# kkromberg/SpeechRecognition

Measured on AMD Instinct MI355X. Metric: frames/sec scored+decoded, higher is better.
Workload: dtype f64

## Files before the change

include/srgpu.h:

```cpp
#ifndef SRGPU_H
#define SRGPU_H

#include <stddef.h>
#include <stdint.h>

#ifdef __cplusplus
extern "C" {
#endif

#if defined(__GNUC__)
#define SR_API __attribute__((visibility("default")))
#else
#define SR_API
#endif

#define SR_ABI_VERSION 4
SR_API int sr_abi_version(void);

#define SR_OK 0
#define SR_EINVAL (-1)
#define SR_EHIP (-2)
#define SR_ENODEV (-3)
#define SR_ELIMIT (-4)
#define SR_ENOMEM (-5)
// ... 192 lines not shown
                                        double posterior_floor, uint32_t max_items, const uint32_t* trans,
                                        const uint64_t* trans_off, double* out_cost, uint16_t* out_count,
                                        uint16_t* out_state, double* out_weight);
SR_API int sr_bigram_mmi_statistics_corpus(sr_model* m, sr_corpus* c, sr_bigram* b, int gmm_kernel, double scale,
                                           double posterior_floor, int max_approx, const uint32_t* trans,
                                           const uint64_t* trans_off, double* out_num_cost, double* out_den_cost,
                                           double* num_mean_acc, double* num_mean_w, double* num_var_acc, double* num_var_w,
                                           double* den_mean_acc, double* den_mean_w, double* den_var_acc, double* den_var_w);


SR_API int sr_bigram_word_lattice_corpus(sr_model* m, sr_corpus* c, sr_bigram* b, int gmm_kernel, double lattice_beam, uint64_t cap,
                                         uint64_t* out_arc_off, double* out_best, uint32_t* out_word, uint32_t* out_hist,
                                         uint32_t* out_pred, uint32_t* out_first, uint32_t* out_last, double* out_fwd, double* out_bwd,
                                         double* out_am);
SR_API int sr_bigram_lattice_nbest(uint32_t n_frames, uint64_t n_arcs, const uint32_t* word, const uint32_t* hist,
                                   const uint32_t* first, const uint32_t* last, const double* am, uint32_t n_words,
                                   uint32_t silence_word, const float* lm, double lm_scale, uint32_t n_best, uint32_t* out_words,
                                   uint64_t words_cap, uint64_t* out_off, double* out_cost, uint32_t* out_count);

typedef struct sr_bigram_stream sr_bigram_stream;
SR_API int sr_bigram_stream_open(sr_model* m, sr_bigram* b, const sr_bigram_params* p, uint32_t max_streams, uint64_t max_frames,
                                 sr_bigram_stream** out);
SR_API int sr_bigram_stream_begin(sr_bigram_stream* s, uint32_t* id);
SR_API int sr_bigram_stream_push(sr_bigram_stream* s, uint32_t n, const uint32_t* ids, const float* feats, const uint64_t* frame_off);
SR_API int sr_bigram_stream_partial(sr_bigram_stream* s, uint32_t id, uint32_t* out_word, float* out_score, uint32_t* out_time,
                                    uint32_t cap, uint32_t* count, uint64_t* frames);
SR_API int sr_bigram_stream_end(sr_bigram_stream* s, uint32_t id, uint32_t* out_word, float* out_score, uint32_t* out_time,
                                uint32_t cap, uint32_t* count);
SR_API int sr_bigram_stream_destroy(sr_bigram_stream* s);

SR_API int sr_probe_fp16_denormals(int device, int* preserved);
SR_API int sr_probe_fp16_accumulation(int device, int* within_model, double* worst_ratio);

typedef struct {
  double gmm_ms;
  uint64_t gmm_launches;
  double gmm_flops;
  double search_ms;
  uint64_t search_launches;
  double search_bytes;
  uint64_t frames;
  uint64_t refined_pairs;
  uint64_t refined_densities;
  double prefilter_ms;
  double refine_ms;
} sr_profile;
SR_API int sr_profile_enable(sr_model* m, int on);
SR_API int sr_profile_reset(sr_model* m);
SR_API int sr_profile_read(sr_model* m, sr_profile* out);

#ifdef __cplusplus
}
#endif
#endif
```

speechrecognition_amd/capi.py:

```python
from __future__ import annotations

import ctypes as C
import os

import numpy as np

HERE = os.path.dirname(os.path.abspath(__file__))
LIB_PATH = os.environ.get("SRGPU_LIB") or os.path.join(HERE, "libsrgpu.so")

GMM_MFMA, GMM_EXACT, GMM_PREFILTER, GMM_DEFAULT = 0, 1, 2, 3
POOL_GLOBAL, POOL_MIXTURE, POOL_NONE = 0, 1, 2
SEARCH_GENERAL_KERNEL = 1
SEARCH_SLOT_KERNEL = 2
BIGRAM_DENSE_STATES = 1
BIGRAM_GLOBAL_STATES = 2
SR_ECORRUPT = -7
SR_ABI_VERSION = 4

SYMBOLS = [
    "sr_abi_version", "sr_model_trim",
    "sr_last_error", "sr_device_count", "sr_model_create", "sr_model_load_mixset", "sr_model_destroy", "sr_model_info",
    "sr_corpus_upload", "sr_corpus_upload_async", "sr_corpus_wait", "sr_corpus_destroy", "sr_shard_utterances", "sr_recognize_batch_multi", "sr_score_corpus", "sr_score_frames", "sr_lexicon_create",
    "sr_lexicon_destroy", "sr_lexicon_describe", "sr_recognize_corpus", "sr_traceback_corpus", "sr_traceback_words", "sr_recognize_batch", "sr_align_corpus", "sr_align_corpus_pruned", "sr_path_scores_corpus", "sr_model_create_from_statistics", "sr_model_create_from_accumulated", "sr_mixset_write", "sr_model_set_tying", "sr_model_tying_info", "sr_model_topology", "sr_accumulate_corpus",
    "sr_state_posteriors_corpus", "sr_baum_welch_corpus", "sr_word_posteriors_corpus", "sr_recognize_confidence_corpus",
    "sr_net_occupancies_corpus", "sr_mmi_statistics_corpus", "sr_model_create_from_mmi_statistics",
    "sr_smbr_max_positions", "sr_net_accuracies_corpus", "sr_smbr_statistics_corpus",
    "sr_word_lattice_corpus", "sr_lattice_nbest",
    "sr_fmllr_statistics_corpus", "sr_fmllr_statistics_bw_corpus", "sr_fmllr_estimate", "sr_corpus_transform",
    "sr_bigram_create", "sr_bigram_destroy", "sr_bigram_describe", "sr_recognize_bigram_corpus",
    "sr_bigram_word_posteriors_corpus", "sr_recognize_bigram_confidence_corpus",
    "sr_bigram_occupancies_corpus", "sr_bigram_mmi_statistics_corpus",
    "sr_bigram_word_lattice_corpus", "sr_bigram_lattice_nbest",
    "sr_stream_open", "sr_stream_begin", "sr_stream_push", "sr_stream_partial", "sr_stream_end", "sr_stream_destroy",
    "sr_bigram_stream_open", "sr_bigram_stream_begin", "sr_bigram_stream_push", "sr_bigram_stream_partial", "sr_bigram_stream_end",
    "sr_bigram_stream_destroy",
    "sr_probe_fp16_denormals", "sr_probe_fp16_accumulation",
    "sr_profile_enable", "sr_profile_reset", "sr_profile_read",
]


class SrError(RuntimeError):
    def __init__(self, code, msg):
        super().__init__(f"libsrgpu error {code}: {msg}")
        self.code = code


def smbr_max_positions():
    n = C.c_uint32()
    _check(lib().sr_smbr_max_positions(C.byref(n)))
    return n.value


class SearchParams(C.Structure):
    _fields_ = [("am_threshold", C.c_double), ("word_penalty", C.c_double), ("gmm_kernel", C.c_int), ("flags", C.c_int)]


class BigramParams(C.Structure):
    _fields_ = [("acoustic_pruning", C.c_float), ("lm_pruning", C.c_float), ("gmm_kernel", C.c_int), ("max_word_ends", C.c_uint32), ("flags", C.c_int)]


class Profile(C.Structure):
    _fields_ = [("gmm_ms", C.c_double), ("gmm_launches", C.c_uint64), ("gmm_flops", C.c_double),
                ("search_ms", C.c_double), ("search_launches", C.c_uint64), ("search_bytes", C.c_double),
                ("frames", C.c_uint64), ("refined_pairs", C.c_uint64), ("refined_densities", C.c_uint64),
                ("prefilter_ms", C.c_double), ("refine_ms", C.c_double)]


_lib = None

# ... 49 lines not shown
        L.sr_recognize_confidence_corpus.argtypes = [vp, vp, vp, C.POINTER(SearchParams), dbl, vp, vp, vp, vp, vp]
        L.sr_net_occupancies_corpus.argtypes = [vp, vp, vp, C.POINTER(SearchParams), dbl, dbl, u32, vp, vp, vp, vp, vp, vp]
        L.sr_mmi_statistics_corpus.argtypes = [vp, vp, vp, C.POINTER(SearchParams), dbl, dbl, i32, vp, vp] + [vp] * 10
        L.sr_smbr_max_positions.argtypes = [vp]
        L.sr_net_accuracies_corpus.argtypes = [vp, vp, vp, C.POINTER(SearchParams), dbl, dbl, u32, vp, vp, vp, vp, vp, vp]
        L.sr_smbr_statistics_corpus.argtypes = [vp, vp, vp, C.POINTER(SearchParams), dbl, dbl, i32, vp] + [vp] * 10
        L.sr_model_create_from_mmi_statistics.argtypes = [vp] + [vp] * 8 + [dbl, dbl, dbl, C.POINTER(vp)]
        L.sr_word_lattice_corpus.argtypes = [vp, vp, vp, C.POINTER(SearchParams), dbl, u64, vp, vp, vp, vp, vp, vp, vp, vp]
        L.sr_lattice_nbest.argtypes = [u32, u64, vp, vp, vp, vp, u32, u32, vp, u64, vp, vp, C.POINTER(u32)]
        L.sr_bigram_create.argtypes = [vp, u32, vp, vp, u32, vp, vp, C.POINTER(vp)]
        L.sr_bigram_destroy.argtypes = [vp]
        L.sr_bigram_describe.argtypes = [vp, C.c_char_p, C.c_size_t]
        L.sr_recognize_bigram_corpus.argtypes = [vp, vp, vp, C.POINTER(BigramParams), vp, vp, vp, vp]
        L.sr_bigram_word_posteriors_corpus.argtypes = [vp, vp, vp, i32, dbl, dbl, u32, vp, vp, vp, vp]
        L.sr_bigram_occupancies_corpus.argtypes = [vp, vp, vp, i32, dbl, dbl, u32, vp, vp, vp, vp, vp, vp]
        L.sr_bigram_mmi_statistics_corpus.argtypes = [vp, vp, vp, i32, dbl, dbl, i32, vp, vp] + [vp] * 10
        L.sr_recognize_bigram_confidence_corpus.argtypes = [vp, vp, vp, C.POINTER(BigramParams), dbl, vp, vp, vp, vp, vp]
        L.sr_bigram_word_lattice_corpus.argtypes = [vp, vp, vp, i32, dbl, u64] + [vp] * 10
        L.sr_bigram_lattice_nbest.argtypes = [u32, u64, vp, vp, vp, vp, vp, u32, u32, vp, dbl, u32, vp, u64, vp, vp, C.POINTER(u32)]
        L.sr_stream_open.argtypes = [vp, vp, C.POINTER(SearchParams), u32, u64, C.POINTER(vp)]
        L.sr_stream_begin.argtypes = [vp, C.POINTER(u32)]
        L.sr_stream_push.argtypes = [vp, u32, vp, vp, vp]
        L.sr_stream_partial.argtypes = [vp, u32, vp, u32, C.POINTER(u32), C.POINTER(u64)]
        L.sr_stream_end.argtypes = [vp, u32, vp, u32, C.POINTER(u32), vp, vp, vp]
        L.sr_stream_destroy.argtypes = [vp]
        L.sr_bigram_stream_open.argtypes = [vp, vp, C.POINTER(BigramParams), u32, u64, C.POINTER(vp)]
        L.sr_bigram_stream_begin.argtypes = [vp, C.POINTER(u32)]
        L.sr_bigram_stream_push.argtypes = [vp, u32, vp, vp, vp]
        L.sr_bigram_stream_partial.argtypes = [vp, u32, vp, vp, vp, u32, C.POINTER(u32), C.POINTER(u64)]
        L.sr_bigram_stream_end.argtypes = [vp, u32, vp, vp, vp, u32, C.POINTER(u32)]
        L.sr_bigram_stream_destroy.argtypes = [vp]
        L.sr_probe_fp16_denormals.argtypes = [i32, C.POINTER(i32)]
        L.sr_probe_fp16_accumulation.argtypes = [i32, C.POINTER(i32), C.POINTER(dbl)]
        L.sr_profile_enable.argtypes = [vp, i32]
        L.sr_profile_reset.argtypes = [vp]
        L.sr_profile_read.argtypes = [vp, C.POINTER(Profile)]
        _lib = L
    return _lib


def _check(rc):
    if rc != 0:
        raise SrError(rc, lib().sr_last_error().decode(errors="replace"))


def device_count():
    n = C.c_int(0)
    _check(lib().sr_device_count(C.byref(n)))
    return n.value


def _ptr(a):
    return a.ctypes.data if a is not None else None


class Model:

    def __init__(self, handle):
        self.h = handle
        d, s, c = C.c_uint32(), C.c_uint32(), C.c_uint64()
        _check(lib().sr_model_info(self.h, C.byref(d), C.byref(s), C.byref(c)))
        self.dim, self.n_states, self.n_densities = d.value, s.value, c.value

    @classmethod
    def from_mixset(cls, path, dim, pooling=POOL_NONE, max_approx=True, device=0):
        h = C.c_void_p()
# ... 50 lines not shown
        self.close()

    def score_frames(self, feats, kernel=GMM_PREFILTER):
        feats = np.ascontiguousarray(feats, dtype=np.float32)
        out = np.empty((feats.shape[0], self.n_states), dtype=np.float64)
        _check(lib().sr_score_frames(self.h, _ptr(feats), feats.shape[0], kernel, _ptr(out)))
        return out

    def upload(self, feats, frame_off, asynchronous=False):
        return Corpus(self, feats, frame_off, asynchronous)

    def recognize_batch(self, lexicon, feats, frame_off, am_threshold, word_penalty, kernel=GMM_PREFILTER):
        feats = np.ascontiguousarray(feats, dtype=np.float32)
        frame_off = np.ascontiguousarray(frame_off, dtype=np.uint64)
        n = len(frame_off) - 1
        words = np.zeros(max(int(frame_off[-1]), 1), dtype=np.uint32)
        woff = np.zeros(n + 1, dtype=np.uint64)
        sp = SearchParams(am_threshold, word_penalty, kernel, 0)
        _check(lib().sr_recognize_batch(self.h, lexicon.h, C.byref(sp), _ptr(feats), _ptr(frame_off), n, _ptr(words), _ptr(woff)))
        return words[: int(woff[-1])].copy(), woff

    def lexicon(self, word_off, automaton, silence_idx, tdp, silence_state):
        return Lexicon(self, word_off, automaton, silence_idx, tdp, silence_state)

    def bigram(self, word_off, mixtures, silence_word, lm, tdp):
        return Bigram(self, word_off, mixtures, silence_word, lm, tdp)

    def stream(self, lexicon, am_threshold, word_penalty, kernel=GMM_PREFILTER, max_streams=1, max_frames=65535):
        return Stream(self, lexicon, am_threshold, word_penalty, kernel, max_streams, max_frames)

    def bigram_stream(self, bigram, acoustic_pruning=None, lm_pruning=None, kernel=GMM_PREFILTER, max_streams=1, max_frames=65535):
        return BigramStream(self, bigram, FLT_MAX if acoustic_pruning is None else acoustic_pruning,
                            FLT_MAX if lm_pruning is None else lm_pruning, kernel, max_streams, max_frames)

    def profile(self, on=True):
        _check(lib().sr_profile_enable(self.h, int(on)))
        _check(lib().sr_profile_reset(self.h))

    def profile_read(self):
        p = Profile()
        _check(lib().sr_profile_read(self.h, C.byref(p)))
        return {k: getattr(p, k) for k, _ in Profile._fields_}


FLT_MAX = float(np.finfo(np.float32).max)


class Bigram:

    def __init__(self, model, word_off, mixtures, silence_word, lm, tdp):
        self.model = model
        word_off = np.ascontiguousarray(word_off, dtype=np.uint32)
        mixtures = np.ascontiguousarray(mixtures, dtype=np.uint16)
        W = len(word_off) - 1
        lm = np.ascontiguousarray(lm, dtype=np.float32)
        assert lm.shape == (W, W)
        tdp = np.ascontiguousarray(tdp, dtype=np.float32)
        assert tdp.size == 8
        self.h = C.c_void_p()
        _check(lib().sr_bigram_create(model.h, W, _ptr(word_off), _ptr(mixtures), silence_word, _ptr(lm), _ptr(tdp), C.byref(self.h)))

    def describe(self):
        buf = C.create_string_buffer(32)
        _check(lib().sr_bigram_describe(self.h, buf, len(buf)))
        return buf.value.decode()

# ... 545 lines not shown
```

speechrecognition_amd/csrc/gmm_prefilter.hip:

```cpp
#include <hip/hip_runtime.h>
#include <stdint.h>

#include <algorithm>
#include <cmath>
#include <vector>

#include "kernels.h"

#ifndef SR_P16_NB
#define SR_P16_NB 4
#endif

namespace srgpu {

typedef float v4f __attribute__((ext_vector_type(4)));
static constexpr int kPWaves = 4;
static constexpr int kGroupBlocks = 8;

typedef _Float16 f16x8 __attribute__((ext_vector_type(8)));

__device__ inline uint32_t pack_f16x2(_Float16 l, _Float16 h) {
  return (uint32_t)__builtin_bit_cast(uint16_t, l) | ((uint32_t)__builtin_bit_cast(uint16_t, h) << 16);
}

template <int KS32, int NB>
__global__ __launch_bounds__(kPWaves * 64, (NB <= 2 ? 3 : 2)) void gmm_prefilter16_kernel(GmmPrefilterArgs a) {
  constexpr int kBlockBytes = KS32 * 1024;
  constexpr int kStageBytes = kGroupBlocks * kBlockBytes;
  constexpr int kChunksPerStage = kStageBytes / 1024;
  constexpr int kDmaPerWave = kChunksPerStage / kPWaves;
  static_assert(kChunksPerStage % kPWaves == 0, "every wave issues the same number of LDS-DMA pieces per stage");
  constexpr int kTileFrames = kPWaves * NB * 16;
  constexpr size_t kTileBytes = (size_t)kTileFrames * (16 * KS32) * sizeof(float);
  constexpr size_t kLdsBytes = 2 * kStageBytes > kTileBytes ? 2 * kStageBytes : kTileBytes;
  __shared__ __attribute__((aligned(1024))) unsigned char lds[kLdsBytes];

// ... 274 lines not shown
  switch (ks32) {
    case 1: hipLaunchKernelGGL((gmm_prefilter16_kernel<1, SR_P16_NB>), grid, block, 0, stream, a); break;
    case 2: hipLaunchKernelGGL((gmm_prefilter16_kernel<2, SR_P16_NB>), grid, block, 0, stream, a); break;
    case 3: hipLaunchKernelGGL((gmm_prefilter16_kernel<3, SR_P16_NB>), grid, block, 0, stream, a); break;
    case 4: hipLaunchKernelGGL((gmm_prefilter16_kernel<4, SR_P16_NB>), grid, block, 0, stream, a); break;
    default: return hipErrorInvalidValue;
  }
  return hipGetLastError();
}
int gmm_prefilter_frames_per_tile() { return kPWaves * SR_P16_NB * 16; }

#pragma clang fp contract(off)

#ifndef SR_R_THREADS
#define SR_R_THREADS 768
#endif
#ifndef SR_R_BATCH
#define SR_R_BATCH 4
#endif
static constexpr int kRThreads = SR_R_THREADS;
static constexpr int kRThreadsWide = 512;
static constexpr int kRWaves = kRThreads / 64;
static constexpr int kRBatch = SR_R_BATCH;
#ifndef SR_R_BATCH_WIDE
#define SR_R_BATCH_WIDE 8
#endif
static constexpr int kRBatchWide = SR_R_BATCH_WIDE;
static constexpr uint32_t kRingEntries = 128;
static constexpr uint32_t kRingLists = 2 * 8 * kRingEntries;
static constexpr uint32_t kRingWave = 4 * kRingLists;
struct __attribute__((aligned(16))) RingEntry { uint32_t lf, mask; double score; };
struct __attribute__((packed, aligned(4))) RowPiece { float v[4]; };

template <int DT, int NS, int SPW, int CH, int NT = kRThreads, int VS = 1, bool DEFER = false>
__global__ __launch_bounds__(NT) void gmm_refine_kernel(GmmRefineArgs a) {
  static_assert(DT > 0 && (DT & 1), "padded dimension: odd");
  static_assert(!DEFER || CH > 1, "deferred lists: states of several chunks");
  constexpr int kRThreads = NT, kRWaves = NT / 64;
  static_assert(CH == 1 || CH == 2 || CH == 4, "chunks per state (half)");
  static_assert(VS == 1 || (VS == 2 && CH == 4), "two halves only of four-chunk states");
  static_assert(SPW % (CH * VS) == 0 && (CH == 1 || SPW % 4 == 0), "a state's chunks live in one workgroup");
  extern __shared__ __attribute__((aligned(1024))) unsigned char panel_raw[];
  const uint32_t D = (uint32_t)DT, tid = threadIdx.x;
  const int lane = tid & 63, wave = tid >> 6;
  const uint32_t s0 = blockIdx.x * SPW;
  const uint32_t ns = (s0 + SPW <= a.n_pstates) ? SPW : a.n_pstates - s0;
  const uint32_t state_bytes = (2u * D + 2u) * NS * 8u;
  const uint64_t f_begin = (uint64_t)blockIdx.y * a.frames_per_split;
  const uint64_t f_end = (f_begin + a.frames_per_split < a.n_frames) ? f_begin + a.frames_per_split : a.n_frames;

  {
    const uint32_t chunks = (ns * state_bytes + 1023u) >> 10;
    const unsigned char* src = reinterpret_cast<const unsigned char*>(a.rows) + (uint64_t)s0 * state_bytes + lane * 16;
    for (uint32_t ch = wave; ch < chunks; ch += kRWaves)
      __builtin_amdgcn_global_load_lds((const __attribute__((address_space(1))) void*)(src + (uint64_t)ch * 1024u),
                                       (__attribute__((address_space(3))) void*)(panel_raw + ch * 1024u), 16, 0, 0);
  }
  uint32_t nd[SPW];
#pragma unroll
  for (int j = 0; j < SPW; j++) nd[j] = (uint32_t)j < ns ? a.n_dens_ps[s0 + j] : 0u;
  __builtin_amdgcn_s_waitcnt(0x0F70);
  __syncthreads();
  if (f_begin >= f_end) return;

  uint32_t n_eval = 0;
  double x[DT];
  const __amdgpu_buffer_rsrc_t featsT_rsrc = __builtin_amdgcn_make_buffer_rsrc(
      const_cast<float*>(a.featsT), 0, (int)0xFFFFFFFFu, 0x00020000);
  const uint32_t ld4 = (uint32_t)a.n_frames_ld * 4u;
  auto load_x = [&](uint64_t f) __attribute__((always_inline)) {
    const uint32_t voff = (uint32_t)f * 4u;
#pragma unroll
    for (int k = 0; k < DT; k++)
      x[k] = (double)__builtin_bit_cast(float, __builtin_amdgcn_raw_buffer_load_b32(featsT_rsrc, voff, (uint32_t)k * ld4, 0));
  };
  auto load_x_row = [&](uint64_t f) __attribute__((always_inline)) {
    const float* xr = a.feats + f * (uint64_t)DT;
#pragma unroll
    for (int q = 0; q < DT / 4; q++) {
      const RowPiece t = reinterpret_cast<const RowPiece*>(xr)[q];
#pragma unroll
      for (int i = 0; i < 4; i++) x[4 * q + i] = (double)t.v[i];
    }
// ... 485 lines not shown

hipError_t launch_transpose_feats(const float* feats, uint64_t n_frames, uint32_t dim, uint32_t dp, uint64_t ldT, float* out, float* featsP,
                                  hipStream_t stream) {
  if (n_frames == 0) return hipSuccess;
  if (dp < dim || (dp != dim && !featsP)) return hipErrorInvalidValue;
  hipLaunchKernelGGL(transpose_feats_kernel, dim3((unsigned)((n_frames + 63) / 64)), dim3(256), 0, stream, feats, n_frames, dim, dp, ldT, out,
                     dp != dim ? featsP : nullptr);
  return hipGetLastError();
}

int gmm_refine_slots(uint32_t max_dens, uint32_t padded_dim) { return padded_dim > 39 ? 32 : max_dens <= 8 ? 8 : max_dens <= 16 ? 16 : 32; }

uint32_t gmm_refine_padded_dim(uint32_t dim) {
  static const uint32_t bounds[] = {9, 17, 25, 33, 39, 47, 55, 63};
  const uint32_t need = dim | 1u;
  for (uint32_t b : bounds)
    if (need <= b) return b;
  return 0;
}

static int refine_threads(uint32_t dp) { return dp <= 47 ? kRThreads : kRThreadsWide; }
static int refine_spw(const GmmRefineArgs& a) {
  return (size_t)(2 * a.dim + 2) * a.n_slots * 8 * 8 <= 160 * 1024 ? 8 : 4;
}
static void refine_grid(const GmmRefineArgs& a, int spw, uint32_t* n_sgroups, uint64_t* splits, uint64_t* frames_per_split) {
  const uint64_t nt = (uint64_t)refine_threads(a.dim);
  *n_sgroups = (a.n_pstates + spw - 1) / spw;
  uint64_t sp = std::max<uint64_t>(1, (512 + *n_sgroups - 1) / *n_sgroups);
  sp = std::min<uint64_t>(sp, (a.n_frames + nt - 1) / nt);
  sp = std::max<uint64_t>(sp, 1);
  *frames_per_split = (a.n_frames + sp - 1) / sp;
  *splits = *frames_per_split ? (a.n_frames + *frames_per_split - 1) / *frames_per_split : 1;
}
size_t gmm_refine_ring_words(const GmmRefineArgs& a) {
  uint32_t g; uint64_t sp, fps;
  refine_grid(a, refine_spw(a), &g, &sp, &fps);
  return (size_t)g * sp * kRWaves * kRingWave;
}

static uint32_t defer_cap_for(const GmmRefineArgs& a, int spw) {
  uint32_t g; uint64_t sp, fps;
  refine_grid(a, spw, &g, &sp, &fps);
  const uint64_t per_wave = ((fps + kRThreads - 1) / kRThreads) * 64;
  return (uint32_t)std::min<uint64_t>(((per_wave / 4 + 63) & ~(uint64_t)63) + 64, 1u << 30);
}
void gmm_refine_defer_layout(const GmmRefineArgs& a, size_t budget_bytes, uint32_t cap_limit, uint32_t* cap, size_t* n_entries,
                             size_t* n_counts) {
  *cap = 0; *n_entries = 0; *n_counts = 0;
  if (a.chunks < 2 || a.dim > 39 || a.n_slots != 32 || a.n_frames == 0) return;
  uint32_t g; uint64_t sp, fps;
  refine_grid(a, 8, &g, &sp, &fps);
  uint32_t c = defer_cap_for(a, 8);
  if (cap_limit) c = std::min(c, cap_limit);
  const size_t segs = (size_t)g * sp * kRWaves * 8;
  if (segs * c * 16 > budget_bytes) return;
  *cap = c; *n_entries = segs * c; *n_counts = segs;
}

template <int DT, int NS, int SPW, int CH, int NT, int VS = 1>
static hipError_t launch_refine_one(const GmmRefineArgs& a0, hipStream_t stream) {
  GmmRefineArgs a = a0;
  const size_t state_bytes = (size_t)(2 * DT + 2) * NS * 8;
  const size_t smem = (SPW * state_bytes + 1023) & ~(size_t)1023;
  uint32_t n_sgroups;
  uint64_t splits;
  refine_grid(a, SPW, &n_sgroups, &splits, &a.frames_per_split);
  const dim3 grid(n_sgroups, (unsigned)splits), block(NT);
  if constexpr (CH > 1 && NT == kRThreads && SPW == 8) {
    if (a.defer && a.defer_cnt && a.defer_cap) {
      auto k1 = gmm_refine_kernel<DT, NS, SPW, CH, NT, VS, true>;
      auto k2 = gmm_drain_kernel<DT, NS, SPW, CH, NT, VS>;
      hipError_t e = hipFuncSetAttribute((const void*)k1, hipFuncAttributeMaxDynamicSharedMemorySize, (int)smem);
      if (e == hipSuccess) e = hipFuncSetAttribute((const void*)k2, hipFuncAttributeMaxDynamicSharedMemorySize, (int)smem);
      if (e != hipSuccess) return e;
      hipLaunchKernelGGL(k1, grid, block, smem, stream, a);
      if ((e = hipGetLastError()) != hipSuccess) return e;
      hipLaunchKernelGGL(k2, grid, block, smem, stream, a);
      return hipGetLastError();
    }
  }
  a.defer = nullptr; a.defer_cnt = nullptr; a.defer_cap = 0;
  auto kernel = gmm_refine_kernel<DT, NS, SPW, CH, NT, VS>;
  hipError_t e = hipFuncSetAttribute((const void*)kernel, hipFuncAttributeMaxDynamicSharedMemorySize, (int)smem);
  if (e != hipSuccess) return e;
  hipLaunchKernelGGL(kernel, grid, block, smem, stream, a);
  return hipGetLastError();
}

template <int DT>
static hipError_t launch_refine_narrow(const GmmRefineArgs& a, hipStream_t stream) {
  switch (a.n_slots) {
    case 8: return launch_refine_one<DT, 8, 8, 1, kRThreads>(a, stream);
    case 16: return launch_refine_one<DT, 16, 8, 1, kRThreads>(a, stream);
    case 32:
      if (a.chunks == 2) return launch_refine_one<DT, 32, 8, 2, kRThreads>(a, stream);
      if (a.chunks == 4) return launch_refine_one<DT, 32, 8, 4, kRThreads>(a, stream);
      if (a.chunks == 8) return launch_refine_one<DT, 32, 8, 4, kRThreads, 2>(a, stream);
      return launch_refine_one<DT, 32, 8, 1, kRThreads>(a, stream);
    default: return hipErrorInvalidValue;
  }
}
template <int DT>
static hipError_t launch_refine_wide(const GmmRefineArgs& a, hipStream_t stream) {
  if (a.n_slots != 32) return hipErrorInvalidValue;
  if (a.chunks == 2) return launch_refine_one<DT, 32, 4, 2, kRThreadsWide>(a, stream);
  if (a.chunks == 4) return launch_refine_one<DT, 32, 4, 4, kRThreadsWide>(a, stream);
  return launch_refine_one<DT, 32, 4, 1, kRThreadsWide>(a, stream);
}

hipError_t launch_gmm_refine(const GmmRefineArgs& a, hipStream_t stream) {
  if (a.n_frames == 0) return hipSuccess;
  if (!a.ring || (uint64_t)a.dim * a.n_frames_ld * 4u >= (1ull << 32)) return hipErrorInvalidValue;
  if (a.chunks != 1 && (a.n_slots != 32 || (a.chunks != 2 && a.chunks != 4 && a.chunks != 8))) return hipErrorInvalidValue;
  if (a.chunks == 8 && a.dim > 39) return hipErrorInvalidValue;
  switch (a.dim) {
    case 9: return launch_refine_narrow<9>(a, stream);
    case 17: return launch_refine_narrow<17>(a, stream);
    case 25: return launch_refine_narrow<25>(a, stream);
    case 33: return launch_refine_narrow<33>(a, stream);
    case 39: return launch_refine_narrow<39>(a, stream);
    case 47:
      if (a.n_slots != 32) return hipErrorInvalidValue;
      return a.chunks == 2 ? launch_refine_one<47, 32, 4, 2, kRThreads>(a, stream) : a.chunks == 4 ? launch_refine_one<47, 32, 4, 4, kRThreads>(a, stream)
                           : launch_refine_one<47, 32, 4, 1, kRThreads>(a, stream);
    case 55: return launch_refine_wide<55>(a, stream);
    case 63: return launch_refine_wide<63>(a, stream);
    default: return hipErrorInvalidValue;
  }
}

}
```

speechrecognition_amd/csrc/kernels.h:

```cpp
#pragma once
#include <hip/hip_runtime.h>
#include <stdint.h>

#include <vector>

namespace srgpu {

struct GmmMfmaArgs {
  const float* feats;
  uint64_t n_frames;
  uint32_t dim;
  const double* apack;
  const uint32_t* blk_meta;
  const uint32_t* grp_state;
  const uint32_t* split_begin;
  double* out;
  uint32_t ld;
  uint32_t nx, ny;
};
int gmm_mfma_ksteps_for_dim(uint32_t dim);
int gmm_mfma_frames_per_tile(int ksteps);
hipError_t launch_gmm_mfma(const GmmMfmaArgs& a, int ksteps, bool sum, hipStream_t stream);

struct GmmExactArgs {
// ... 20 lines not shown
  uint32_t blk_first;
  uint64_t frame_base;
};
hipError_t launch_gmm_exact_listed(const GmmExactArgs& a, bool sum, const GmmExactList& L, uint32_t n_blocks, hipStream_t stream);
int gmm_exact_frames_per_block();

struct GmmPrefilterArgs {
  const float* feats;
  uint64_t n_frames;
  uint32_t dim;
  const unsigned char* apack;
  const float* grp_lim;
  const uint32_t* split_begin;
  uint32_t* mask;
  uint32_t nx, ny;
  uint32_t chunks;
};
struct PfBound { float kappa, acc, abs, sub; };
constexpr float kPfRes16 = 4.8835e-4f;
inline constexpr PfBound pf_bound(int ks32) {
  return ks32 == 4 ? PfBound{1.05e-3f, 1.6e-5f, 7.0e-7f, 3.38e-7f} : PfBound{1.05e-3f, 1.1e-5f, 6.0e-7f, 2.92e-7f};
}
struct GmmRefineArgs {
  const float* feats;
  const float* featsT;
  uint64_t n_frames, n_frames_ld;
  uint32_t dim, n_pstates, chunks;
  const uint32_t* n_dens_ps;
  const double* rows;
  uint32_t n_slots;
  const uint32_t* mask;
  double* out; uint32_t ld;
  uint64_t frames_per_split;
  unsigned long long* n_refined;
  uint32_t* ring;
  void* defer;
  uint32_t* defer_cnt;
  uint32_t defer_cap;
};
void gmm_refine_defer_layout(const GmmRefineArgs& a, size_t budget_bytes, uint32_t cap_limit, uint32_t* cap, size_t* n_entries,
                             size_t* n_counts);
size_t gmm_refine_ring_words(const GmmRefineArgs& a);
hipError_t launch_gmm_prefilter(const GmmPrefilterArgs& a, int ks32, hipStream_t stream);
int gmm_prefilter_frames_per_tile();
hipError_t probe_fp16_denormals(hipStream_t stream, bool* preserved);
hipError_t probe_fp16_accumulation(hipStream_t stream, int ks32, bool* ok, double* worst_ratio);
uint32_t gmm_refine_padded_dim(uint32_t dim);
int gmm_refine_slots(uint32_t max_dens, uint32_t padded_dim);
hipError_t launch_gmm_refine(const GmmRefineArgs& a, hipStream_t stream);
hipError_t launch_transpose_feats(const float* feats, uint64_t n_frames, uint32_t dim, uint32_t dp, uint64_t ldT, float* out, float* featsP,
                                  hipStream_t stream);

struct DecodeNet {
  uint32_t n_slots;
  uint32_t n_words;
  const uint32_t* slot_info;
  const uint32_t* slot_word;
  const uint32_t* word_end_slot;
  uint32_t silence_word;
  double tdp_loop, tdp_forward, tdp_skip;
  uint32_t silence_state;
};
static constexpr uint32_t kSlotPos0 = 1u << 16;
static constexpr uint32_t kSlotPos1 = 1u << 17;
static constexpr uint32_t kSlotEnd = 1u << 18;
static constexpr uint32_t kSlotSilState = 1u << 19;
static constexpr uint32_t kSlotSilWord = 1u << 20;
static constexpr uint32_t kSlotFirstSil = 1u << 21;
static constexpr uint32_t kSlotSingle = 1u << 22;
struct FastNet {
  uint32_t n_slots;
  const uint32_t* state;
  const uint32_t* pred;
  const uint32_t* orig;
  const uint32_t* chunk_type;
// ... 507 lines not shown
```

speechrecognition_amd/csrc/srgpu_api.cpp:

```cpp
#include <hip/hip_runtime.h>

#include <algorithm>
#include <cmath>
#include <cstdarg>
#include <cstdio>
#include <cstdlib>
#include <cstring>
#include <limits>
#include <map>
#include <memory>
#include <mutex>
#include <numeric>
#include <queue>
#include <set>
#include <string>
#include <vector>

#include "../../include/srgpu.h"
#include "host_util.h"
#include "kernels.h"
#include "traceback.h"

using namespace srgpu;
using srhost::guarded;
// ... 3908 lines not shown
  const int64_t slot = s->slots.find(id);
  if (slot < 0) return fail(SR_EINVAL, "stream id %u is not open", id);
  int rc = check_model(s->model);
  if (rc) return rc;
  if (frames) *frames = s->slots.frames[slot];
  return bigram_stream_items(s, (uint32_t)slot, id, out_word, out_score, out_time, cap, count);
  });
}

int sr_bigram_stream_end(sr_bigram_stream* s, uint32_t id, uint32_t* out_word, float* out_score, uint32_t* out_time, uint32_t cap,
                         uint32_t* count) {
  return guarded(__func__, [&]() -> int {
  if (!s || !count || ((!out_word || !out_score || !out_time) && cap)) return fail(SR_EINVAL, "null argument");
  const int64_t slot = s->slots.find(id);
  if (slot < 0) return fail(SR_EINVAL, "stream id %u is not open", id);
  int rc = check_model(s->model);
  if (rc) return rc;
  rc = bigram_stream_items(s, (uint32_t)slot, id, out_word, out_score, out_time, cap, count);
  if (rc == SR_EINVAL) return rc;
  s->slots.open[slot] = 0;
  return rc;
  });
}

int sr_bigram_stream_destroy(sr_bigram_stream* s) {
  return guarded(__func__, [&]() -> int {
  if (!s) return SR_OK;
  if (s->model) { (void)hipSetDevice(s->model->device); (void)hipDeviceSynchronize(); }
  delete s;
  return SR_OK;
  });
}

int sr_profile_enable(sr_model* m, int on) {
  return guarded(__func__, [&]() -> int {
  if (!m) return fail(SR_EINVAL, "null model handle");
  m->profiling = on != 0;
  return SR_OK;
  });
}

int sr_profile_reset(sr_model* m) {
  return guarded(__func__, [&]() -> int {
  int rc = check_model(m);
  if (rc) return rc;
  HIP_TRY(hipDeviceSynchronize());
  for (auto& ep : m->events) { (void)hipEventDestroy(ep.a); (void)hipEventDestroy(ep.b); }
  m->events.clear();
  m->prof = sr_profile{};
  HIP_TRY(m->pf_counter.ensure(1));
  HIP_TRY(hipMemset(m->pf_counter.p, 0, sizeof(unsigned long long)));
  return SR_OK;
  });
}

int sr_profile_read(sr_model* m, sr_profile* out) {
  return guarded(__func__, [&]() -> int {
  int rc = check_model(m);
  if (rc) return rc;
  if (!out) return fail(SR_EINVAL, "out is null");
  HIP_TRY(hipDeviceSynchronize());
  for (auto& ep : m->events) {
    float ms = 0.f;
    HIP_TRY(hipEventElapsedTime(&ms, ep.a, ep.b));
    if (ep.kind == 0) { m->prof.gmm_ms += ms; m->prof.gmm_launches++; }
    else if (ep.kind == 1) { m->prof.search_ms += ms; m->prof.search_launches++; }
// ... 18 lines not shown
```

Baseline: 13.85 million.

## Use persistent occupancy-sized grid dealing state-group passes in GMM refine kernel

For the common refine configuration (32 slots, one chunk, 8 states per workgroup, default thread count), the 2D grid of state groups by frame splits is replaced by a persistent grid sized to occupancy times CU count. Each workgroup takes a contiguous, evenly dealt range of (state group, frame pass) items and loops over the state groups in it, reloading state panels with a barrier between groups. The aim is to remove tail imbalance and launch-shape inefficiency across CUs. In exchange it adds occupancy queries cached per device, scalar index arithmetic in the kernel, and a describe API for inspecting the chosen plan.

```diff
diff --git a/include/srgpu.h b/include/srgpu.h
--- a/include/srgpu.h
+++ b/include/srgpu.h
@@ -248,6 +248,8 @@
 SR_API int sr_probe_fp16_denormals(int device, int* preserved);
 SR_API int sr_probe_fp16_accumulation(int device, int* within_model, double* worst_ratio);
 
+SR_API int sr_refine_describe(sr_model* m, uint64_t n_frames, char* out, size_t cap);
+
 typedef struct {
   double gmm_ms;
   uint64_t gmm_launches;
diff --git a/speechrecognition_amd/capi.py b/speechrecognition_amd/capi.py
--- a/speechrecognition_amd/capi.py
+++ b/speechrecognition_amd/capi.py
@@ -34,7 +34,7 @@
     "sr_stream_open", "sr_stream_begin", "sr_stream_push", "sr_stream_partial", "sr_stream_end", "sr_stream_destroy",
     "sr_bigram_stream_open", "sr_bigram_stream_begin", "sr_bigram_stream_push", "sr_bigram_stream_partial", "sr_bigram_stream_end",
     "sr_bigram_stream_destroy",
-    "sr_probe_fp16_denormals", "sr_probe_fp16_accumulation",
+    "sr_probe_fp16_denormals", "sr_probe_fp16_accumulation", "sr_refine_describe",
     "sr_profile_enable", "sr_profile_reset", "sr_profile_read",
 ]
 
@@ -150,6 +150,7 @@
         L.sr_bigram_stream_destroy.argtypes = [vp]
         L.sr_probe_fp16_denormals.argtypes = [i32, C.POINTER(i32)]
         L.sr_probe_fp16_accumulation.argtypes = [i32, C.POINTER(i32), C.POINTER(dbl)]
+        L.sr_refine_describe.argtypes = [vp, u64, C.c_char_p, C.c_size_t]
         L.sr_profile_enable.argtypes = [vp, i32]
         L.sr_profile_reset.argtypes = [vp]
         L.sr_profile_read.argtypes = [vp, C.POINTER(Profile)]
@@ -266,6 +267,11 @@
     def bigram_stream(self, bigram, acoustic_pruning=None, lm_pruning=None, kernel=GMM_PREFILTER, max_streams=1, max_frames=65535):
         return BigramStream(self, bigram, FLT_MAX if acoustic_pruning is None else acoustic_pruning,
                             FLT_MAX if lm_pruning is None else lm_pruning, kernel, max_streams, max_frames)
+
+    def refine_describe(self, n_frames):
+        buf = C.create_string_buffer(160)
+        _check(lib().sr_refine_describe(self.h, int(n_frames), buf, len(buf)))
+        return buf.value.decode()
 
     def profile(self, on=True):
         _check(lib().sr_profile_enable(self.h, int(on)))
diff --git a/speechrecognition_amd/csrc/gmm_prefilter.hip b/speechrecognition_amd/csrc/gmm_prefilter.hip
--- a/speechrecognition_amd/csrc/gmm_prefilter.hip
+++ b/speechrecognition_amd/csrc/gmm_prefilter.hip
@@ -2,6 +2,7 @@
 #include <stdint.h>
 
 #include <algorithm>
+#include <atomic>
 #include <cmath>
 #include <vector>
 
@@ -342,8 +343,79 @@
 struct __attribute__((aligned(16))) RingEntry { uint32_t lf, mask; double score; };
 struct __attribute__((packed, aligned(4))) RowPiece { float v[4]; };
 
+__device__ inline const GmmRefineArgs& refine_args() {
+  auto p = (const __attribute__((address_space(4))) GmmRefineArgs*)__builtin_amdgcn_kernarg_segment_ptr();
+  asm volatile("" : "+s"(p));
+  return *(const GmmRefineArgs*)p;
+}
+__device__ inline uint32_t refine_workgroup() {
+  uint32_t w = blockIdx.x;
+  asm volatile("" : "+s"(w));
+  return w;
+}
+__device__ inline void refine_range(const GmmRefineArgs& a, uint32_t w, uint32_t* begin, uint32_t* end) {
+  *begin = w * a.deal_q + (uint32_t)__builtin_amdgcn_readfirstlane((int)(w * a.deal_r / gridDim.x));
+  *end = (w + 1u) * a.deal_q + (uint32_t)__builtin_amdgcn_readfirstlane((int)((w + 1u) * a.deal_r / gridDim.x));
+}
+__device__ inline uint32_t refine_group_of(const GmmRefineArgs& a, uint32_t item) {
+  return (uint32_t)__builtin_amdgcn_readfirstlane((int)(item / a.deal_passes));
+}
+__device__ inline uint32_t refine_first_group(const GmmRefineArgs& a) {
+  if (!a.deal_passes) return blockIdx.x;
+  uint32_t b, e;
+  refine_range(a, refine_workgroup(), &b, &e);
+  return refine_group_of(a, b);
+}
+__device__ inline bool refine_last_group(const GmmRefineArgs& a, uint32_t g) {
+  if (!a.deal_passes) return true;
+  uint32_t b, e;
+  refine_range(a, refine_workgroup(), &b, &e);
+  return g >= refine_group_of(a, e - 1u);
+}
+template <int NT>
+__device__ inline void refine_visit(const GmmRefineArgs& a, uint32_t g, uint64_t* f_begin, uint64_t* f_end, uint32_t* visit) {
+  if (a.deal_passes) {
+    uint32_t b, e;
+    refine_range(a, refine_workgroup(), &b, &e);
+    const uint32_t i0 = g * a.deal_passes, i1 = i0 + a.deal_passes;
+    *f_begin = (uint64_t)((b > i0 ? b : i0) - i0) * NT;
+    const uint64_t fe = (uint64_t)((e < i1 ? e : i1) - i0) * NT;
+    *f_end = fe < a.n_frames ? fe : a.n_frames;
+    *visit = g - refine_group_of(a, b);
+  } else {
+    *f_begin = (uint64_t)blockIdx.y * a.frames_per_split;
+    *f_end = (*f_begin + a.frames_per_split < a.n_frames) ? *f_begin + a.frames_per_split : a.n_frames;
+    *visit = 0;
+  }
+}
+
+template <int DT, int NS, int SPW, int CH, int NT, int VS, bool DEFER>
+__device__ __forceinline__ void gmm_refine_group(const GmmRefineArgs& a, const uint32_t s0, const uint64_t f_begin, const uint64_t f_end,
+                                                 const uint32_t visit);
 template <int DT, int NS, int SPW, int CH, int NT = kRThreads, int VS = 1, bool DEFER = false>
-__global__ __launch_bounds__(NT) void gmm_refine_kernel(GmmRefineArgs a) {
+__global__ __launch_bounds__(NT) void gmm_refine_kernel(GmmRefineArgs args) {
+  if constexpr (DEFER || !(NS == 32 && CH == 1 && NT == 768 && SPW == 8)) {
+    uint64_t f_begin, f_end;
+    uint32_t visit;
+    refine_visit<NT>(args, blockIdx.x, &f_begin, &f_end, &visit);
+    gmm_refine_group<DT, NS, SPW, CH, NT, VS, DEFER>(args, blockIdx.x * SPW, f_begin, f_end, 0u);
+  } else {
+    uint32_t g = refine_first_group(refine_args());
+#pragma unroll 1
+    for (;; g++) {
+      uint64_t f_begin, f_end;
+      uint32_t visit;
+      const GmmRefineArgs& a = refine_args();
+      refine_visit<NT>(a, g, &f_begin, &f_end, &visit);
+      gmm_refine_group<DT, NS, SPW, CH, NT, VS, DEFER>(a, g * SPW, f_begin, f_end, visit);
+      if (refine_last_group(refine_args(), g)) break;
+    }
+  }
+}
+
+template <int DT, int NS, int SPW, int CH, int NT, int VS, bool DEFER>
+__device__ __forceinline__ void gmm_refine_group(const GmmRefineArgs& a, const uint32_t s0, const uint64_t f_begin, const uint64_t f_end,
+                                                 const uint32_t visit) {
   static_assert(DT > 0 && (DT & 1), "padded dimension: odd");
   static_assert(!DEFER || CH > 1, "deferred lists: states of several chunks");
   constexpr int kRThreads = NT, kRWaves = NT / 64;
@@ -353,12 +425,10 @@
   extern __shared__ __attribute__((aligned(1024))) unsigned char panel_raw[];
   const uint32_t D = (uint32_t)DT, tid = threadIdx.x;
   const int lane = tid & 63, wave = tid >> 6;
-  const uint32_t s0 = blockIdx.x * SPW;
   const uint32_t ns = (s0 + SPW <= a.n_pstates) ? SPW : a.n_pstates - s0;
   const uint32_t state_bytes = (2u * D + 2u) * NS * 8u;
-  const uint64_t f_begin = (uint64_t)blockIdx.y * a.frames_per_split;
-  const uint64_t f_end = (f_begin + a.frames_per_split < a.n_frames) ? f_begin + a.frames_per_split : a.n_frames;
-
+
+  if (visit) __syncthreads();
   {
     const uint32_t chunks = (ns * state_bytes + 1023u) >> 10;
     const unsigned char* src = reinterpret_cast<const unsigned char*>(a.rows) + (uint64_t)s0 * state_bytes + lane * 16;
@@ -910,40 +980,84 @@
   *frames_per_split = (a.n_frames + sp - 1) / sp;
   *splits = *frames_per_split ? (a.n_frames + *frames_per_split - 1) / *frames_per_split : 1;
 }
+
+struct RefinePlan {
+  uint32_t n_sgroups;
+  uint64_t splits, frames_per_split;
+  uint32_t deal_wgs, deal_passes, deal_visits;
+  uint64_t deal_items;
+  uint64_t wave_frames;
+  uint32_t workgroups() const { return deal_wgs ? deal_wgs : (uint32_t)(n_sgroups * splits); }
+};
+static uint32_t refine_deal_width(const GmmRefineArgs& a);
+static RefinePlan refine_plan(const GmmRefineArgs& a, int spw) {
+  RefinePlan p{};
+  refine_grid(a, spw, &p.n_sgroups, &p.splits, &p.frames_per_split);
+  const uint64_t nt = (uint64_t)refine_threads(a.dim);
+  p.wave_frames = ((p.frames_per_split + nt - 1) / nt) * 64;
+  if (spw == 8 && a.n_slots == 32 && a.chunks == 1 && nt == (uint64_t)kRThreads && a.n_frames >= nt && a.n_frames < (1ull << 30)) {
+    const uint64_t passes = (a.n_frames + nt - 1) / nt, items = p.n_sgroups * passes;
+    const uint32_t w = items >= 2 ? refine_deal_width(a) : 0;
+    if (w && w < 65536u && items >= 2ull * w && items < (1ull << 31)) {
+      p.deal_items = items;
+      const uint64_t most = (items + w - 1) / w;
+      p.deal_wgs = w;
+      p.deal_passes = (uint32_t)passes;
+      p.deal_visits = (uint32_t)((most + passes - 1) / passes) + 1;
+      p.wave_frames = most * 64;
+    }
+  }
+  return p;
+}
 size_t gmm_refine_ring_words(const GmmRefineArgs& a) {
-  uint32_t g; uint64_t sp, fps;
-  refine_grid(a, refine_spw(a), &g, &sp, &fps);
-  return (size_t)g * sp * kRWaves * kRingWave;
-}
-
-static uint32_t defer_cap_for(const GmmRefineArgs& a, int spw) {
-  uint32_t g; uint64_t sp, fps;
-  refine_grid(a, spw, &g, &sp, &fps);
-  const uint64_t per_wave = ((fps + kRThreads - 1) / kRThreads) * 64;
-  return (uint32_t)std::min<uint64_t>(((per_wave / 4 + 63) & ~(uint64_t)63) + 64, 1u << 30);
-}
+  return (size_t)refine_plan(a, refine_spw(a)).workgroups() * kRWaves * kRingWave;
+}
+void gmm_refine_describe(const GmmRefineArgs& a, uint32_t* workgroups, uint32_t* deal_passes, uint32_t* deal_visits) {
+  const RefinePlan p = refine_plan(a, refine_spw(a));
+  *workgroups = p.workgroups(); *deal_passes = p.deal_passes; *deal_visits = p.deal_visits;
+}
+
 void gmm_refine_defer_layout(const GmmRefineArgs& a, size_t budget_bytes, uint32_t cap_limit, uint32_t* cap, size_t* n_entries,
                              size_t* n_counts) {
   *cap = 0; *n_entries = 0; *n_counts = 0;
   if (a.chunks < 2 || a.dim > 39 || a.n_slots != 32 || a.n_frames == 0) return;
-  uint32_t g; uint64_t sp, fps;
-  refine_grid(a, 8, &g, &sp, &fps);
-  uint32_t c = defer_cap_for(a, 8);
+  const RefinePlan p = refine_plan(a, 8);
+  uint32_t c = (uint32_t)std::min<uint64_t>(((p.wave_frames / 4 + 63) & ~(uint64_t)63) + 64, 1u << 30);
   if (cap_limit) c = std::min(c, cap_limit);
-  const size_t segs = (size_t)g * sp * kRWaves * 8;
+  const size_t segs = (size_t)p.workgroups() * kRWaves * 8;
   if (segs * c * 16 > budget_bytes) return;
   *cap = c; *n_entries = segs * c; *n_counts = segs;
 }
 
 template <int DT, int NS, int SPW, int CH, int NT, int VS = 1>
-static hipError_t launch_refine_one(const GmmRefineArgs& a0, hipStream_t stream) {
+static hipError_t launch_refine_one(const GmmRefineArgs& a0, hipStream_t stream, uint32_t* width) {
   GmmRefineArgs a = a0;
   const size_t state_bytes = (size_t)(2 * DT + 2) * NS * 8;
   const size_t smem = (SPW * state_bytes + 1023) & ~(size_t)1023;
-  uint32_t n_sgroups;
-  uint64_t splits;
-  refine_grid(a, SPW, &n_sgroups, &splits, &a.frames_per_split);
-  const dim3 grid(n_sgroups, (unsigned)splits), block(NT);
+  constexpr bool kDeal = NS == 32 && CH == 1 && NT == kRThreads && SPW == 8;
+  auto kernel = gmm_refine_kernel<DT, NS, SPW, CH, NT, VS>;
+  if (width) {
+    *width = 0;
+    if constexpr (kDeal) {
+      static std::atomic<uint32_t> known[64];
+      int dev = 0, cus = 0;
+      hipError_t e = hipGetDevice(&dev);
+      if (e != hipSuccess) return e;
+      if (dev >= 0 && dev < 64 && known[dev].load(std::memory_order_relaxed)) { *width = known[dev].load(std::memory_order_relaxed); return hipSuccess; }
+      if ((e = hipDeviceGetAttribute(&cus, hipDeviceAttributeMultiprocessorCount, dev)) != hipSuccess) return e;
+      int per_cu = 0;
+      if ((e = hipFuncSetAttribute((const void*)kernel, hipFuncAttributeMaxDynamicSharedMemorySize, (int)smem)) != hipSuccess) return e;
+      if ((e = hipOccupancyMaxActiveBlocksPerMultiprocessor(&per_cu, (const void*)kernel, NT, smem)) != hipSuccess) return e;
+      if (per_cu > 0 && cus > 0) *width = (uint32_t)per_cu * (uint32_t)cus;
+      if (dev >= 0 && dev < 64) known[dev].store(*width, std::memory_order_relaxed);
+    }
+    return hipSuccess;
+  }
+  const RefinePlan p = refine_plan(a, SPW);
+  a.frames_per_split = p.frames_per_split;
+  a.deal_passes = p.deal_passes;
+  if (p.deal_wgs) { a.deal_q = (uint32_t)(p.deal_items / p.deal_wgs); a.deal_r = (uint32_t)(p.deal_items % p.deal_wgs); }
+  const dim3 grid = p.deal_wgs ? dim3(p.deal_wgs) : dim3(p.n_sgroups, (unsigned)p.splits), block(NT);
   if constexpr (CH > 1 && NT == kRThreads && SPW == 8) {
     if (a.defer && a.defer_cnt && a.defer_cap) {
       auto k1 = gmm_refine_kernel<DT, NS, SPW, CH, NT, VS, true>;
@@ -958,7 +1072,6 @@
     }
   }
   a.defer = nullptr; a.defer_cnt = nullptr; a.defer_cap = 0;
-  auto kernel = gmm_refine_kernel<DT, NS, SPW, CH, NT, VS>;
   hipError_t e = hipFuncSetAttribute((const void*)kernel, hipFuncAttributeMaxDynamicSharedMemorySize, (int)smem);
   if (e != hipSuccess) return e;
   hipLaunchKernelGGL(kernel, grid, block, smem, stream, a);
@@ -966,45 +1079,52 @@
 }
 
 template <int DT>
-static hipError_t launch_refine_narrow(const GmmRefineArgs& a, hipStream_t stream) {
+static hipError_t launch_refine_narrow(const GmmRefineArgs& a, hipStream_t stream, uint32_t* width) {
   switch (a.n_slots) {
-    case 8: return launch_refine_one<DT, 8, 8, 1, kRThreads>(a, stream);
-    case 16: return launch_refine_one<DT, 16, 8, 1, kRThreads>(a, stream);
+    case 8: return launch_refine_one<DT, 8, 8, 1, kRThreads>(a, stream, width);
+    case 16: return launch_refine_one<DT, 16, 8, 1, kRThreads>(a, stream, width);
     case 32:
-      if (a.chunks == 2) return launch_refine_one<DT, 32, 8, 2, kRThreads>(a, stream);
-      if (a.chunks == 4) return launch_refine_one<DT, 32, 8, 4, kRThreads>(a, stream);
-      if (a.chunks == 8) return launch_refine_one<DT, 32, 8, 4, kRThreads, 2>(a, stream);
-      return launch_refine_one<DT, 32, 8, 1, kRThreads>(a, stream);
+      if (a.chunks == 2) return launch_refine_one<DT, 32, 8, 2, kRThreads>(a, stream, width);
+      if (a.chunks == 4) return launch_refine_one<DT, 32, 8, 4, kRThreads>(a, stream, width);
+      if (a.chunks == 8) return launch_refine_one<DT, 32, 8, 4, kRThreads, 2>(a, stream, width);
+      return launch_refine_one<DT, 32, 8, 1, kRThreads>(a, stream, width);
     default: return hipErrorInvalidValue;
   }
 }
 template <int DT>
-static hipError_t launch_refine_wide(const GmmRefineArgs& a, hipStream_t stream) {
+static hipError_t launch_refine_wide(const GmmRefineArgs& a, hipStream_t stream, uint32_t* width) {
   if (a.n_slots != 32) return hipErrorInvalidValue;
-  if (a.chunks == 2) return launch_refine_one<DT, 32, 4, 2, kRThreadsWide>(a, stream);
-  if (a.chunks == 4) return launch_refine_one<DT, 32, 4, 4, kRThreadsWide>(a, stream);
-  return launch_refine_one<DT, 32, 4, 1, kRThreadsWide>(a, stream);
-}
-
+  if (a.chunks == 2) return launch_refine_one<DT, 32, 4, 2, kRThreadsWide>(a, stream, width);
+  if (a.chunks == 4) return launch_refine_one<DT, 32, 4, 4, kRThreadsWide>(a, stream, width);
+  return launch_refine_one<DT, 32, 4, 1, kRThreadsWide>(a, stream, width);
+}
+
+static hipError_t dispatch_refine(const GmmRefineArgs& a, hipStream_t stream, uint32_t* width) {
+  if (a.chunks != 1 && (a.n_slots != 32 || (a.chunks != 2 && a.chunks != 4 && a.chunks != 8))) return hipErrorInvalidValue;
+  if (a.chunks == 8 && a.dim > 39) return hipErrorInvalidValue;
+  switch (a.dim) {
+    case 9: return launch_refine_narrow<9>(a, stream, width);
+    case 17: return launch_refine_narrow<17>(a, stream, width);
+    case 25: return launch_refine_narrow<25>(a, stream, width);
+    case 33: return launch_refine_narrow<33>(a, stream, width);
+    case 39: return launch_refine_narrow<39>(a, stream, width);
+    case 47:
+      if (a.n_slots != 32) return hipErrorInvalidValue;
+      return a.chunks == 2 ? launch_refine_one<47, 32, 4, 2, kRThreads>(a, stream, width) : a.chunks == 4 ? launch_refine_one<47, 32, 4, 4, kRThreads>(a, stream, width)
+                           : launch_refine_one<47, 32, 4, 1, kRThreads>(a, stream, width);
+    case 55: return launch_refine_wide<55>(a, stream, width);
+    case 63: return launch_refine_wide<63>(a, stream, width);
+    default: return hipErrorInvalidValue;
+  }
+}
+static uint32_t refine_deal_width(const GmmRefineArgs& a) {
+  uint32_t w = 0;
+  return dispatch_refine(a, nullptr, &w) == hipSuccess ? w : 0u;
+}
 hipError_t launch_gmm_refine(const GmmRefineArgs& a, hipStream_t stream) {
   if (a.n_frames == 0) return hipSuccess;
   if (!a.ring || (uint64_t)a.dim * a.n_frames_ld * 4u >= (1ull << 32)) return hipErrorInvalidValue;
-  if (a.chunks != 1 && (a.n_slots != 32 || (a.chunks != 2 && a.chunks != 4 && a.chunks != 8))) return hipErrorInvalidValue;
-  if (a.chunks == 8 && a.dim > 39) return hipErrorInvalidValue;
-  switch (a.dim) {
-    case 9: return launch_refine_narrow<9>(a, stream);
-    case 17: return launch_refine_narrow<17>(a, stream);
-    case 25: return launch_refine_narrow<25>(a, stream);
-    case 33: return launch_refine_narrow<33>(a, stream);
-    case 39: return launch_refine_narrow<39>(a, stream);
-    case 47:
-      if (a.n_slots != 32) return hipErrorInvalidValue;
-      return a.chunks == 2 ? launch_refine_one<47, 32, 4, 2, kRThreads>(a, stream) : a.chunks == 4 ? launch_refine_one<47, 32, 4, 4, kRThreads>(a, stream)
-                           : launch_refine_one<47, 32, 4, 1, kRThreads>(a, stream);
-    case 55: return launch_refine_wide<55>(a, stream);
-    case 63: return launch_refine_wide<63>(a, stream);
-    default: return hipErrorInvalidValue;
-  }
-}
-
-}
+  return dispatch_refine(a, stream, nullptr);
+}
+
+}
diff --git a/speechrecognition_amd/csrc/kernels.h b/speechrecognition_amd/csrc/kernels.h
--- a/speechrecognition_amd/csrc/kernels.h
+++ b/speechrecognition_amd/csrc/kernels.h
@@ -76,6 +76,8 @@
   const uint32_t* mask;
   double* out; uint32_t ld;
   uint64_t frames_per_split;
+  uint32_t deal_passes;
+  uint32_t deal_q, deal_r;
   unsigned long long* n_refined;
   uint32_t* ring;
   void* defer;
@@ -85,6 +87,7 @@
 void gmm_refine_defer_layout(const GmmRefineArgs& a, size_t budget_bytes, uint32_t cap_limit, uint32_t* cap, size_t* n_entries,
                              size_t* n_counts);
 size_t gmm_refine_ring_words(const GmmRefineArgs& a);
+void gmm_refine_describe(const GmmRefineArgs& a, uint32_t* workgroups, uint32_t* deal_passes, uint32_t* deal_visits);
 hipError_t launch_gmm_prefilter(const GmmPrefilterArgs& a, int ks32, hipStream_t stream);
 int gmm_prefilter_frames_per_tile();
 hipError_t probe_fp16_denormals(hipStream_t stream, bool* preserved);
diff --git a/speechrecognition_amd/csrc/srgpu_api.cpp b/speechrecognition_amd/csrc/srgpu_api.cpp
--- a/speechrecognition_amd/csrc/srgpu_api.cpp
+++ b/speechrecognition_amd/csrc/srgpu_api.cpp
@@ -3964,6 +3964,25 @@
   });
 }
 
+int sr_refine_describe(sr_model* m, uint64_t n_frames, char* out, size_t cap) {
+  return guarded(__func__, [&]() -> int {
+  int rc = check_model(m);
+  if (rc) return rc;
+  if (!out || cap == 0) return fail(SR_EINVAL, "null argument");
+  if ((rc = reserve_scoring(m, SR_GMM_PREFILTER, 0))) return rc;
+  if (resolve_dense_kernel(m, SR_GMM_PREFILTER) != SR_GMM_PREFILTER || m->pf_ks32 == 0 || n_frames == 0) {
+    snprintf(out, cap, "none");
+    return SR_OK;
+  }
+  uint32_t wgs = 0, passes = 0, visits = 0;
+  gmm_refine_describe(refine_shape(m, n_frames), &wgs, &passes, &visits);
+  const DeferLayout dl = defer_layout(m, n_frames);
+  if (passes) snprintf(out, cap, "deal %u workgroups, %u passes per group, %u groups at most, deferred %u", wgs, passes, visits, dl.cap);
+  else snprintf(out, cap, "grid %u workgroups, deferred %u", wgs, dl.cap);
+  return SR_OK;
+  });
+}
+
 int sr_profile_enable(sr_model* m, int on) {
   return guarded(__func__, [&]() -> int {
   if (!m) return fail(SR_EINVAL, "null model handle");
```

After: 13.75 million. Within noise of the previous version (-0.8%).
